# haampie/Homogenization.jl

Hardware: AMD Instinct MI355X
Metric: fine-DOF updates/sec per V-cycle (3D Tet64) (higher is better)
Workload: dtype f64; 1 GPU; 3D Tet64 checkerboard, 32^3 unit cubes x 6 tets, refinements=5 (BASELINE config 3); cells=196608, nf=6545, levels=6, smoothing_steps=3, smoothing_steps_coarse=2, coarse_solver=device CG, Chebyshev(4)-of-Jacobi preconditioner, rtol 1e-13, spare_vector_bytes=10294394880, lazy_top_form=2

## Files before the change

homogenization.jl_amd/csrc/hmg_apply.hip:

```cpp
#include "hmg_apply_launch.hpp"
#include "hmg_device.hpp"
#include "hmg_stencil.hpp"

#include <cstdio>
#include <stdexcept>
#include <string>

namespace hmg {

#ifdef HMG_PHASE_TIMING
#define HMG_STAMP(i)                                                                     \
    do {    \
        if (a.blockpart && !a.cell_list && tid == 0)                                     \
            a.blockpart[2 * (size_t)a.nwork + 8 * cell + (i)] = (double)wall_clock64(); \
    } while (0)
#define HMG_SLAB_T0() const long long _t0 = wall_clock64(); long long _tl = _t0; double _ph[5] = {0, 0, 0, 0, 0}
#define HMG_SLAB_PHASE(i)                              \
    do {                                               \
        const long long _n = wall_clock64();           \
        _ph[i] += (double)(_n - _tl);                  \
        _tl = _n;                                      \
    } while (0)
#define HMG_SLAB_STORE()                                                                      \
    do {                                                                                      \
// ... 1083 lines not shown
    throw std::runtime_error("operator apply: no instantiation for this shape and role");
}

void launch_apply(const Launch &L, const LevelDev &lv, const MeshDev &mesh, double alpha, double lambda,
                  const double *x, const double *src, double *out, int use_mask)
{
    ApplyArgs a{};
    a.alpha = alpha;
    a.lambda = lambda;
    a.x = x;
    a.src = src;
    a.out = out;
    a.flags = (use_mask ? 1 : 0) | (L.apply_mass_only ? 2 : 0);
#ifdef HMG_PHASE_TIMING
    a.blockpart = mesh.blockpart;
#endif
    if (lv.dim == 3)
        launch_apply_dim<3, false>(L, lv, mesh, a);
    else
        launch_apply_dim<2, false>(L, lv, mesh, a);
}

void launch_apply_args(const Launch &L, const LevelDev &lv, const MeshDev &mesh, ApplyArgs a)
{
    a.flags = (a.flags & 1) | (L.apply_mass_only ? 2 : 0);
    if (lv.dim == 3)
        launch_apply_dim<3, false>(L, lv, mesh, a);
    else
        launch_apply_dim<2, false>(L, lv, mesh, a);
}

void launch_apply_fused_kernel(const Launch &L, const LevelDev &lv, const MeshDev &mesh, ApplyArgs a)
{
    a.scal = L.scal;
    if (!(a.flags & 32)) a.mult = mesh.mult;
    a.blockpart = mesh.blockpart;
    if (a.flags & 8) {
        if (lv.dim == 3)
            launch_apply_dim<3, true, true>(L, lv, mesh, a);
        else
            launch_apply_dim<2, true, true>(L, lv, mesh, a);
        return;
    }
    if (lv.dim == 3)
        launch_apply_dim<3, true>(L, lv, mesh, a);
    else
        launch_apply_dim<2, true>(L, lv, mesh, a);
}

void launch_apply_fused_reduce(const Launch &L, const MeshDev &mesh, int slot_pap, int slot_rr)
{
    hipLaunchKernelGGL(k_reduce_pairs, dim3(256), dim3(256), 0, L.stream, mesh.blockpart, mesh.ncells, L.partials);
    check_launch();
    launch_finalize(L, L.partials, 256, slot_pap);
    if (slot_rr >= 0)
        launch_finalize(L, L.partials + 2048, 256, slot_rr);
    check_launch();
}

void launch_restrict_slab(const Launch &L, const LevelDev &fine_rtab, const MeshDev &mesh, const SlabTables &st,
                          int ldc, const double *rf, double *bc)
{
    ApplyArgs a{};
    a.alpha = 1.0;
    a.x = rf;
    a.out = bc;
    a.out_ld = ldc;
// ... 35 lines not shown
```

homogenization.jl_amd/csrc/hmg_context.cpp:

```cpp
#include "../../include/hmg.h"
#include "hmg_objects.hpp"

#include <algorithm>

namespace hmg {

std::recursive_mutex &lifetime_mutex()
{
    static std::recursive_mutex m;
    return m;
}

std::atomic<int64_t> &device_allocs()
{
    static std::atomic<int64_t> n{0};
    return n;
}

namespace {

void vec_pool_trim(hmg_ctx *c)
{
    LifetimeLock lock(lifetime_mutex());
    if (c->vec_pool.empty()) return;
// ... 78 lines not shown
    c->L.rpart_cap = need_blocks;
}

void ctx_unref(hmg_ctx *ctx)
{
    LifetimeLock lock(lifetime_mutex());
    if (!ctx || --ctx->refs > 0) return;
    auto &lc = live_contexts();
    lc.erase(std::remove(lc.begin(), lc.end(), ctx), lc.end());
    (void)hipSetDevice(ctx->device);
    (void)hipStreamSynchronize(ctx->stream);
    for (auto &ev : ctx->timer.pool) {
        (void)hipEventDestroy(ev.first);
        (void)hipEventDestroy(ev.second);
    }
    vec_pool_trim(ctx);
    comm_drop(ctx);
    if (ctx->own_stream) (void)hipStreamDestroy(ctx->stream);
    delete ctx;
}

}

void grid_unref(hmg_grid *grid)
{
    LifetimeLock lock(lifetime_mutex());
    if (!grid || --grid->refs > 0) return;
    hmg_ctx *c = grid->ctx;
    if (c) {
        (void)hipSetDevice(c->device);
        (void)hipStreamSynchronize(c->stream);
    }
    probe_unlist(grid);
    release_top_spare(grid);
    release_weight_cache(grid);
    release_smoother_diag(grid);
    if (grid->probe && grid->probe->h) (void)hipHostFree(grid->probe->h);
    if (grid->probe && grid->probe->ev) (void)hipEventDestroy(grid->probe->ev);
    delete grid;
    ctx_unref(c);
}

void release_vec(hmg_vec *v)
{
    if (v->own && v->d) vec_release(v->g->ctx, v->d, v->bytes);
    hmg_grid *g = v->g;
    delete v;
    grid_unref(g);
}

double read_scalar(hmg_ctx *c, int slot)
{
    double h = 0.0;
    HIPCHK(hipMemcpyAsync(&h, c->L.scal + slot, sizeof(double), hipMemcpyDeviceToHost, c->stream));
    HIPCHK(hipStreamSynchronize(c->stream));
    judge_probes(c);
    return h;
}

}

extern "C" {

const char *hmg_last_error(void) { return last_error().c_str(); }
int hmg_version(void) { return 1; }

// ... 66 lines not shown
int hmg_ctx_sync(hmg_ctx *ctx)
{
    HMG_TRY
    need(ctx != nullptr, "null ctx");
    HIPCHK(hipStreamSynchronize(ctx->stream));
    judge_probes(ctx);
    HMG_END
}

int64_t hmg_ctx_counter(hmg_ctx *ctx, const char *name)
{
    if (!ctx || !name) return -1;
    const std::string n(name);
    if (n == "wave_launches") return ctx->wave_launches;
    if (n == "slab2_launches") return ctx->slab2_launches;
    if (n == "rows_launches") return ctx->rows_launches;
    if (n == "small_launches") return ctx->small_launches;
    if (n == "weight_cache_launches") return ctx->wc_launches;
    if (n == "comm_calls") return ctx->comm_calls;
    if (n == "device_allocs") return device_allocs().load();
    if (n == "spare_bytes") return ctx->spare_bytes;
    if (n == "weight_cache_classes") return ctx->wc_classes;
    if (n == "weight_cache_bytes") return ctx->wc_bytes;
    if (n == "weight_cache_refusals") return ctx->wc_refusals;
    if (n == "fcg_bytes") return ctx->fcg_bytes;
    if (n == "smoother_diag_bytes") return ctx->smoother_diag_bytes;
    if (n == "smoother_diag_builds") return ctx->smoother_diag_builds;
    if (n == "lazy_top_form") return ctx->last_top_form;
    if (n == "lazy_pre_form") return ctx->last_pre_form;
    if (n == "lazy_r_form") return ctx->last_r_form;
    if (n == "r_materialized") return ctx->r_materialized;
    if (n == "r_materialized_by_read") return ctx->r_materialized_read;
    if (n == "r_dropped") return ctx->r_dropped;
    if (n == "coarse_x_folds") return ctx->coarse_x_folds;
    if (n == "cell_moments_kernel_ns") return ctx->moments_kernel_ns;
    if (n == "cell_moments_download_ns") return ctx->moments_download_ns;
    if (n == "cell_pair_moments_kernel_ns") return ctx->pair_moments_kernel_ns;
    if (n == "cell_pair_moments_download_ns") return ctx->pair_moments_download_ns;
    if (n == "cell_moments_window_launches") return ctx->moments_window_launches;
    if (n == "cell_moments_windows") return ctx->moments_windows;
    if (n == "cell_extrema_kernel_ns") return ctx->extrema_kernel_ns;
    if (n == "cell_extrema_window_launches") return ctx->extrema_window_launches;
    if (n == "cell_extrema_windows") return ctx->extrema_windows;
    if (n == "comm_nranks") return ctx->comm ? ctx->comm_nranks : 0;
    return -1;
}

int hmg_ctx_release_memory(hmg_ctx *ctx)
{
    HMG_TRY
    need(ctx != nullptr, "null ctx");
    vec_pool_trim(ctx);
    HMG_END
}

int hmg_ctx_set_option(hmg_ctx *ctx, const char *name, int64_t value)
{
    HMG_TRY
    need(ctx && name, "null argument");
    std::string n(name);
    static const std::pair<const char *, bool hmg_ctx::*> flags[] = {
        {"coarse_probe", &hmg_ctx::coarse_probe}, {"fuse_cg", &hmg_ctx::fuse_cg_default}, {"fold_x", &hmg_ctx::fold_x},
        {"swap_rp", &hmg_ctx::swap_rp}, {"fold_prolong", &hmg_ctx::fold_prolong}, {"zero_entry", &hmg_ctx::zero_entry},
        {"fold_restrict", &hmg_ctx::fold_restrict}, {"lazy_dead", &hmg_ctx::lazy_dead}, {"lazy_pre", &hmg_ctx::lazy_pre}, {"fold_coarse_x", &hmg_ctx::fold_coarse_x}, {"fold_faces", &hmg_ctx::fold_faces},
        {"lean_post", &hmg_ctx::lean_post}, {"lazy_post", &hmg_ctx::lazy_post}, {"lazy_r", &hmg_ctx::lazy_r}, {"prolong_in_image", &hmg_ctx::prolong_in_image},
        {"comm_rehearsal", &hmg_ctx::comm_rehearsal}};
    for (const auto &f : flags)
        if (n == f.first) {
            ctx->*f.second = value != 0;
            return 0;
        }
    if (n == "apply_threads")
        ctx->L.apply_threads = (int)value;
    else if (n == "apply_wg512")
        ctx->L.apply_wg512 = value != 0;
    else if (n == "apply_pack")
        ctx->L.apply_pack = value != 0;
    else if (n == "apply_small")
        ctx->L.apply_small = value != 0;
    else if (n == "weight_cache")
        ctx->L.weight_cache = value != 0;
    else if (n == "weight_cache_classes")
        ctx->wc_max_classes = std::max<int64_t>(0, value);
    else if (n == "apply_slab2")
        ctx->L.apply_slab2 = value != 0;
    else if (n == "restrict_slab2")
        ctx->L.restrict_slab2 = value != 0;
    else if (n == "slab2_force")
        ctx->L.slab2_force = value != 0;
    else if (n == "slab2_grid")
        ctx->L.slab2_grid = std::max<int64_t>(0, value);
    else if (n == "apply_wave")
        ctx->L.apply_wave = value != 0;
    else if (n == "wave_grid")
        ctx->L.wave_grid = std::max<int64_t>(1, value) * (int64_t)ctx->L.num_cu;
    else if (n == "wave_grid_total")
        ctx->L.wave_grid = std::max<int64_t>(1, value);
    else if (n == "cell_order")
// ... 174 lines not shown
```

homogenization.jl_amd/csrc/hmg_kernels.hip:

```cpp
#include "hmg_device.hpp"
#include "hmg_stencil.hpp"

#include <cstdio>
#include <stdexcept>
#include <string>

namespace hmg {

__global__ void __launch_bounds__(256) k_finalize(const double *__restrict__ partials, int n, double *scal, int slot)
{
    __shared__ double red[4];
    double v = 0.0;
    for (int i = threadIdx.x; i < n; i += 256) v += partials[i];
    double s = block_sum(v, red);
    if (threadIdx.x == 0) scal[slot] = s;
}

void launch_finalize(const Launch &L, const double *partials, int n, int slot)
{
    hipLaunchKernelGGL(k_finalize, dim3(1), dim3(256), 0, L.stream, partials, n, L.scal, slot);
}

__global__ void __launch_bounds__(256)
k_iface_faces(const int32_t *__restrict__ pairs, int64_t npairs, int nfi, int off_face, int ld, double *x)
// ... 556 lines not shown
    }
    const double s = block_sum(acc, red);
    if (threadIdx.x == 0) partials[blockIdx.x] = s;
}

template <int XU>
__global__ void __launch_bounds__(SB)
k_cg_x_tail(double *x, const double *__restrict__ p, const double *__restrict__ p0, const double *__restrict__ r, int64_t n,
            const double *__restrict__ scal, int s_num, int s_den, XUSlots xs, double *alpha_out)
{
    static_assert(XU == 1 || XU == 2, "one or two stored directions");
    const double alpha = scal[s_num] / scal[s_den];
    const double ax = scal[xs.a_num] / scal[xs.a_den];
    const double beta = scal[xs.b_num] / scal[xs.b_den];
    const double az = XU == 2 ? scal[xs.z_num] / scal[xs.z_den] : 0.0;
    const int64_t i = (int64_t)blockIdx.x * SB + threadIdx.x;
    if (i < (n >> 1)) {
        double2 xv = reinterpret_cast<double2 *>(x)[i];
        const double2 pv = reinterpret_cast<const double2 *>(p)[i];
        const double2 rv = reinterpret_cast<const double2 *>(r)[i];
        if (XU == 2) {
            const double2 zv = reinterpret_cast<const double2 *>(p0)[i];
            xv.x = axpy1(az, zv.x, xv.x);
            xv.y = axpy1(az, zv.y, xv.y);
        }
        xv.x = xupd2(ax, beta, alpha, xv.x, pv.x, rv.x);
        xv.y = xupd2(ax, beta, alpha, xv.y, pv.y, rv.y);
        reinterpret_cast<double2 *>(x)[i] = xv;
    }
    if (blockIdx.x == 0 && threadIdx.x == 0) {
        if (n & 1) x[n - 1] = xupd2(ax, beta, alpha, XU == 2 ? axpy1(az, p0[n - 1], x[n - 1]) : x[n - 1], p[n - 1], r[n - 1]);
        alpha_out[0] = alpha;
        alpha_out[1] = 1.0;
    }
}

__global__ void __launch_bounds__(SB)
k_cg_xp_update(double *x, double *p, const double *__restrict__ r, int64_t n, const double *__restrict__ scal,
               int a_num, int a_den, int s_num, int s_den, int with_p)
{
    const double alpha = scal[a_num] / scal[a_den];
    const double beta = with_p ? scal[s_num] / scal[s_den] : 0.0;
    const int64_t i = (int64_t)blockIdx.x * SB + threadIdx.x;
    if (i < (n >> 1)) {
        double2 *x2 = reinterpret_cast<double2 *>(x);
        double2 *p2 = reinterpret_cast<double2 *>(p);
        double2 xv = x2[i], pv = p2[i];
        double2 rv = make_double2(0.0, 0.0);
        if (with_p) rv = reinterpret_cast<const double2 *>(r)[i];
        xv.x = axpy1(alpha, pv.x, xv.x);
        xv.y = axpy1(alpha, pv.y, xv.y);
        x2[i] = xv;
        if (with_p) {
            pv.x = axpy1(beta, pv.x, rv.x);
            pv.y = axpy1(beta, pv.y, rv.y);
            p2[i] = pv;
        }
    }
    if ((n & 1) && blockIdx.x == 0 && threadIdx.x == 0) {
        x[n - 1] = axpy1(alpha, p[n - 1], x[n - 1]);
        if (with_p) p[n - 1] = axpy1(beta, p[n - 1], r[n - 1]);
    }
}

__global__ void __launch_bounds__(SB)
k_cg_x2_update(double *x, const double *__restrict__ p, const double *__restrict__ r, int64_t n, const double *__restrict__ scal,
// ... 740 lines not shown
```

homogenization.jl_amd/csrc/hmg_objects.hpp:

```cpp
#pragma once

#include "../../include/hmg.h"
#include "hmg_device.hpp"
#include "hmg_host.hpp"

#include <atomic>
#include <memory>
#include <mutex>
#include <stdexcept>
#include <string>
#include <vector>

struct ncclComm;

using namespace hmg;

#define HIPCHK(expr)                                                                            \
    do {                                                                                        \
        hipError_t _e = (expr);                                                                 \
        if (_e != hipSuccess)                                                                   \
            throw std::runtime_error(std::string("HIP error: ") + hipGetErrorString(_e) + " (" #expr ")"); \
    } while (0)

namespace hmg {
// ... 112 lines not shown
    std::vector<double> ev_bytes;
    size_t used = 0;
};

struct FieldState {
    std::vector<ElementTables> elem;
    std::vector<std::unique_ptr<DevBuf<uint8_t>>> d_mask;
};

struct CoarseProbe {
    double *h = nullptr;
    hipEvent_t ev = nullptr;
    bool pending = false;
    int budget = 0;
    int generation = 0;
};

}

struct hmg_ctx {
    int refs = 1;
    ApplyTimer timer;
    bool fuse_cg_default = true;
    bool fold_x = true;
    bool swap_rp = true;
    bool fold_prolong = true;
    bool lazy_dead = true;
    bool lazy_pre = true;
    bool fold_faces = true;
    bool lean_post = true;
    bool lazy_post = true;
    bool fold_coarse_x = true;
    bool lazy_r = true;
    int lazy_top = 2;
    bool zero_entry = true;
    bool fold_restrict = true;
    bool prolong_in_image = true;
    int device = 0;
    hipStream_t stream = nullptr;
    bool own_stream = false;
    DevBuf<double> partials, scal, rpart;
    Launch L{};
    int coarse_maxit = 5000;
    int coarse_check = 25;
    bool coarse_probe = true;
    double coarse_rtol = 1e-13;
    int coarse_poly = 4;
    double coarse_poly_ratio = 20.0;
    ncclComm *comm = nullptr;
    int comm_nranks = 1, comm_rank = 0;
    hipStream_t comm_stream = nullptr;
    hipEvent_t ev_packed = nullptr, ev_summed = nullptr;
    int64_t comm_calls = 0, comm_doubles = 0;
    int64_t small_launches = 0;
    int64_t wc_launches = 0;
    int64_t wave_launches = 0;
    int64_t slab2_launches = 0;
    int64_t rows_launches = 0;
    int64_t wc_max_classes = 0;
    int64_t wc_classes = 0, wc_bytes = 0;
    int64_t wc_refusals = 0;
    int64_t spare_bytes = 0;
    int64_t fcg_bytes = 0;
    int64_t smoother_diag_bytes = 0;
    int64_t smoother_diag_builds = 0;
    int64_t moments_kernel_ns = 0, moments_download_ns = 0;
    int64_t pair_moments_kernel_ns = 0, pair_moments_download_ns = 0;
    int64_t extrema_kernel_ns = 0;
    int moments_windows = 0;
    int64_t moments_window_launches = 0;
    int extrema_windows = 0;
    int64_t extrema_window_launches = 0;
    int64_t coarse_x_folds = 0;
    int last_pre_form = 0;
    int last_r_form = 0;
    int64_t r_materialized = 0;
    int64_t r_materialized_read = 0;
    int64_t r_dropped = 0;
    int last_top_form = 0;
    bool vec_pool_on = true;
    std::vector<std::pair<size_t, void *>> vec_pool;
    bool comm_rehearsal = false;
    int64_t overlap_min_doubles = 524288;
    std::vector<struct hmg_grid *> probe_grids;
};

struct PendingR {
    hmg_vec *r = nullptr, *Ap = nullptr;
    int level = 0;
    int slot = -1;
    bool formed = false;
    bool orphan_Ap = false;
};

struct hmg_grid {
    int refs = 1;
    hmg_ctx *ctx = nullptr;
    int dim = 0, nlevels = 0;
    std::vector<LevelTables> lt;
    std::vector<std::unique_ptr<LevelBufs>> lb;
    std::vector<LevelDev> ld;
    MeshTables mesh_full, mesh;
    bool shrunk = false;
    bool dir_custom = false;
    std::vector<int32_t> dir_faces;
    MeshDev md{};
    DevBuf<int32_t> d_cells, d_face_pairs, d_face_partner, d_edge_ptr, d_edge_ent, d_node_ptr, d_node_ent, d_node_first;
    DevBuf<uint16_t> d_dmask, d_dupmask;
    DevBuf<uint8_t> d_mult;
    DevBuf<double> d_blockpart;
    PendingR pend;
    bool r_reader = false;
    double *pend_alpha() const { return d_blockpart.p ? d_blockpart.p + d_blockpart.n - 2 : nullptr; }
    bool fuse_cg = true;
    DevBuf<double> d_coef;
    std::vector<double> sigma, coef;
    int sig_n = 0;
    DevBuf<int32_t> d_cell_class;
    DevBuf<double> d_coef_rep;
    int nclasses = 0;
    std::vector<int32_t> cell_class;
    int64_t wc_limit = 0;
    bool wc_trim = false;
    int64_t wc_counted_classes = 0, wc_counted_bytes = 0;
    double wc_lambda = 0.0;
    bool wc_ready = false;
    double lambda = 0.0;
    bool has_op = false;
    uint64_t op_epoch = 0;
    CoarseMatrix cm;
    CoarseDev cd{};
    bool coarse_ready = false;
    DevBuf<int32_t> c_rowptr, c_colidx, c_interior;
    DevBuf<double> c_val, c_diag, c_b, c_x, c_r, c_z, c_p, c_q, c_u, c_z2, c_d;
    DevBuf<double> top_spare;
    bool top_spare_refused = false;
    int smoother = 0;
    std::vector<std::unique_ptr<DevBuf<double>>> dinv;
    bool dinv_ready = false;
    std::vector<char> dinv_level_ready;
    bool dinv_build_counted = false;
    double c_lmax = 2.0;
    int coarse_last_it = 0;
    int coarse_budget = 0;
    int coarse_generation = 0;
    int64_t coarse_misses = 0;
// ... 48 lines not shown
{
    last_error() = e.what();
    return 1;
}

#define HMG_TRY try {
#define HMG_END                      \
    }                                \
    catch (const std::exception &e)  \
    {                                \
        return fail(e);              \
    }                                \
    catch (...)                      \
    {                                \
        last_error() = "unknown error"; \
        return 1;                    \
    }                                \
    return 0;

inline void need(bool c, const char *msg)
{
    if (!c) throw std::runtime_error(msg);
}

inline const LevelDev &lev(const hmg_grid *g, int level)
{
    need(g != nullptr, "null grid");
    need(g->ctx != nullptr, "this grid was created without a device context (host tables only): no compute path exists on the CPU");
    need(level >= 1 && level <= g->nlevels, "level out of range");
    return g->ld[level - 1];
}

void materialize_r(hmg_grid *g, bool read = false);
inline void settle(const hmg_vec *v)
{
    if (v && v->g && v->g->pend.r && (v == v->g->pend.r || v == v->g->pend.Ap)) materialize_r(v->g, true);
}
void settle_overwritten(const hmg_vec *v);
bool pending_keeps(hmg_vec *v);

inline void check_vec(const hmg_grid *g, int level, const hmg_vec *v, const char *name, bool settle_pending = true)
{
    if (!v) throw std::runtime_error(std::string("null vector: ") + name);
    if (v->g != g) throw std::runtime_error(std::string("vector belongs to another grid: ") + name);
    if (v->level != level) throw std::runtime_error(std::string("vector has the wrong level: ") + name);
    if (v->alloc_cells < g->md.ncells) throw std::runtime_error(std::string("vector too small: ") + name);
    if (settle_pending) settle(v);
}

inline int64_t vec_len(const hmg_vec *v) { return (int64_t)v->g->ld[v->level - 1].ld * v->g->md.ncells; }

inline bool has_exchange(const hmg_grid *g) { return g->exchange || g->ex_begin || g->p2p || g->p2p_begin; }

double *vec_alloc(hmg_ctx *c, size_t bytes);
void vec_release(hmg_ctx *c, void *p, size_t bytes);
void release_vec(hmg_vec *v);
void grid_unref(hmg_grid *grid);
double read_scalar(hmg_ctx *c, int slot);

void ensure_weight_cache(hmg_grid *g);
void release_weight_cache(hmg_grid *g);

SlabTables slab_tables(const hmg_grid *g, const LevelDev &lv);

void set_slab(hmg_grid *g, const LevelDev &lv);
void apply(hmg_grid *g, const LevelDev &lv, double alpha, const double *x, const double *src, double *out, int mask);
// ... 24 lines not shown
```

homogenization.jl_amd/csrc/hmg_smooth.cpp:

```cpp
#include "../../include/hmg.h"
#include "hmg_objects.hpp"
#include "hmg_pcg.hpp"

#include <algorithm>
#include <cmath>

namespace hmg {

void set_slab(hmg_grid *g, const LevelDev &lv)
{
    const LevelBufs &B = *g->lb[lv.level - 1];
    g->md.slab.head = B.slab_head.p;
    g->md.slab.ld_word = B.slab_ld_word.p;
    g->md.slab.cp_word = B.slab_cp_word.p;
    g->md.slab.cp_slot = B.slab_cp_slot.p;
    g->md.slab.nslab = B.nslab;
    g->md.slab.lds_nodes = B.slab_lds_nodes;
    g->md.slab.max_surf = B.slab_max_surf;
    g->md.slab.max_int = B.slab_max_int;
}

namespace {

struct TimedRegion {
// ... 397 lines not shown
            a.out = Ap->d;
            a.flags = 1;
            apply_then_sum(g, lv, a, true, S_PAP, -1);
        } else {
            apply(g, lv, 1.0, p->d, nullptr, Ap->d, 1);
            interface_sum(g, lv, Ap->d);
            launch_dot(L, p->d, Ap->d, n, S_PAP);
            scalar_sum(g, S_PAP, 1);
        }
        const bool last = i == steps - 1;
        if (last && f.tail != Tail::Full) {
            if (f.tail == Tail::ScratchP) {
                launch_pcg_rupdate(L, r->d, Ap->d, dinv, n, cur, S_PAP, other);
                scalar_sum(g, other, 1);
            }
            launch_cg_xp_update(L, x->d, p->d, r->d, n, cur, S_PAP, cur, other, 0);
            return;
        }
        launch_pcg_rupdate(L, r->d, Ap->d, dinv, n, cur, S_PAP, other);
        scalar_sum(g, other, 1);
        launch_pcg_xp(L, x->d, p->d, r->d, dinv, n, cur, S_PAP, other, cur);
        std::swap(cur, other);
    }
}

bool lazy_r_ok(const hmg_grid *g, const hmg_vec *r, const hmg_vec *p, const hmg_vec *Ap)
{
    if (!g->ctx->lazy_r || g->smoother != 0 || g->part || has_exchange(g) || g->scalar_sum) return false;
    for (const hmg_vec *v : {r, p, Ap})
        if (!v->own || v->exposed) return false;
    return r != Ap && g->pend_alpha() != nullptr && vec_len(r) > 0;
}

void open_pending(hmg_grid *g, int level, hmg_vec *r, hmg_vec *Ap, int slot, bool formed)
{
    LifetimeLock lock(lifetime_mutex());
    need(!g->pend.r, "a pending r-update was not settled before the next one");
    g->pend.r = r;
    g->pend.Ap = Ap;
    g->pend.level = level;
    g->pend.slot = slot;
    g->pend.formed = formed;
    g->ctx->last_r_form = formed ? 0 : 1;
}

DeferredX smooth(hmg_grid *g, int level, int steps, hmg_vec *x, hmg_vec *b, hmg_vec *r, hmg_vec *p, hmg_vec *Ap,
                 const SmoothForm &f, const hmg_vec *xcoarse = nullptr, const DeferredX *cx = nullptr)
{
    const LevelDev &lv = lev(g, level);
    const Launch &L = g->ctx->L;
    const int64_t n = vec_len(x);
    first_residual(g, level, x, b, r, f, xcoarse, cx);
    if (g->smoother == 1) {
        smooth_pcg(g, level, steps, x, r, p, Ap, f);
        return {};
    }
    int cur = S_RS, other = S_RS2;
    if (!g->fuse_cg || steps <= 0) {
        launch_copy_dot(L, p->d, r->d, n, cur);
        scalar_sum(g, cur, 1);
        for (int i = 0; i < steps; ++i) {
            apply(g, lv, 1.0, p->d, nullptr, Ap->d, 1);
            interface_sum(g, lv, Ap->d);
            launch_dot(L, p->d, Ap->d, n, S_PAP);
            scalar_sum(g, S_PAP, 1);
            const bool last = i == steps - 1;
            if (last && f.tail == Tail::DeadXp) {
                launch_cg_xp_update(L, x->d, p->d, r->d, n, cur, S_PAP, cur, other, 0);
                return {};
            }
            launch_cg_update(L, x->d, r->d, p->d, Ap->d, n, cur, S_PAP, other);
            scalar_sum(g, other, 1);
            if (last && f.tail == Tail::ScratchP) return {};
            launch_cg_pupdate(L, p->d, r->d, n, other, cur);
            std::swap(cur, other);
        }
        return {};
    }
    auto args = [&](int i) {
        ApplyArgs a{};
        a.alpha = 1.0;
        a.lambda = g->lambda;
        a.x = r->d;
        a.x2 = i == 0 ? nullptr : p->d;
// ... 72 lines not shown
        }
        return DeferredX{cur, S_PAP2, true, other, S_PAP, cur, other};
    case Tail::DeadDefer3:
        a.x2 = g->top_spare.p;
        a.out = a.xout = a.xacc = nullptr;
        a.s_num = S_RS3;
        a.s_den = cur;
        apply_then_sum(g, lv, a, true, S_PAP3, -1);
        {
            DeferredX d{S_RS3, S_PAP3, true, cur, S_PAP2, S_RS3, cur};
            d.three_updates = true;
            d.d_num = other;
            d.d_den = S_PAP;
            return d;
        }
    case Tail::Top2:
        a.xout = a.xacc = nullptr;
        apply_then_sum(g, lv, a, true, S_PAP2, -1, true, false);
        if (f.lazy_r && !g->r_reader) {
            launch_cg_x_tail(L, r->d, n, cur, S_PAP2, x->d, p->d, other, S_PAP, cur, other, nullptr, 0, 0, g->pend_alpha());
            open_pending(g, level, r, Ap, other, false);
            return {};
        }
        launch_cg_rupdate_faces_x(L, lv, g->md, r->d, r->d, Ap->d, n, cur, S_PAP2, other, x->d, p->d, other, S_PAP, cur, other,
                                  nullptr, 0, 0);
        scalar_sum(g, other, 1);
        if (f.lazy_r) open_pending(g, level, r, Ap, other, true);
        return {};
    case Tail::Top3:
        a.x2 = g->top_spare.p;
        a.xout = a.xacc = nullptr;
        a.s_num = S_RS3;
        a.s_den = cur;
        apply_then_sum(g, lv, a, true, S_PAP3, -1, true, false);
        if (f.lazy_r && !g->r_reader) {
            launch_cg_x_tail(L, r->d, n, S_RS3, S_PAP3, x->d, g->top_spare.p, cur, S_PAP2, S_RS3, cur, p->d, other, S_PAP, g->pend_alpha());
            open_pending(g, level, r, Ap, other, false);
            return {};
        }
        launch_cg_rupdate_faces_x(L, lv, g->md, r->d, r->d, Ap->d, n, S_RS3, S_PAP3, other, x->d, g->top_spare.p, cur, S_PAP2,
                                  S_RS3, cur, p->d, other, S_PAP);
        scalar_sum(g, other, 1);
        if (f.lazy_r) open_pending(g, level, r, Ap, other, true);
        return {};
    }
    return {};
}

bool zero_entry_ok(const hmg_grid *g, int k, int steps)
{
    if (!g->ctx->zero_entry) return false;
    if (k == 1) return true;
    if (g->smoother == 1) return false;
    if (steps != 2 || smooth_form(g, k, steps, Role::Pre).tail != Tail::DeadDefer2) return false;
    const LevelDev &lv = g->ld[k - 1];
    if (lv.blk_R > 0) return g->ctx->fold_restrict && apply_restricts(g->ctx->L, lv);
    return true;
}

int vcycle_down(hmg_grid *g, int k, int steps, hmg_vec **st, bool inside = false, bool x_zero = false, int steps_next = -1)
{
    hmg_vec **cur = st + 5 * (k - 1);
    hmg_vec **nxt = st + 5 * (k - 2);
    const Launch &L = g->ctx->L;
    SmoothForm form = smooth_form(g, k, steps, Role::Pre);
    need(!x_zero || form.tail == Tail::DeadDefer2, "zero initial guess: the pre-smoother does not defer both x-updates");
// ... 55 lines not shown
    const bool fold_p = g->ctx->fold_prolong && g->fuse_cg && apply_lds_bytes(lev(g, k)) <= 160 * 1024 &&
                        apply_lds_bytes(lev(g, k)) + sizeof(double) * (size_t)lev(g, k - 1).nf <= 80 * 1024;
    need(!(cx && cx->rs >= 0) || fold_p, "pending coarse x-updates without the folded prolongation");
    if (!fold_p) launch_prolong_add(L, lev(g, k), lev(g, k - 1), g->md.ncells, nxt[0]->d, cur[0]->d);
    SmoothForm form = smooth_form(g, k, steps, role);
    form.hand_up = hand_up && form.tail == Tail::DeadX2;
    form.lazy_r = lazy_r && (form.tail == Tail::Top2 || form.tail == Tail::Top3) && lazy_r_ok(g, cur[2], cur[3], cur[4]);
    return smooth(g, k, steps, cur[0], cur[1], cur[2], cur[3], cur[4], form, fold_p ? nxt[0] : nullptr, cx);
}

bool coarse_x_folds(const hmg_grid *g, int k, int steps_below)
{
    const hmg_ctx *c = g->ctx;
    if (k < 3 || g->smoother == 1 || !c->fold_coarse_x || !c->lazy_post || !c->fold_prolong || !c->lean_post || !g->fuse_cg || !c->prolong_in_image) return false;
    const LevelDev &lv = g->ld[(size_t)k - 1];
    if (!(apply_lds_bytes(lv) > 48 * 1024 && apply_lds_bytes(lv) <= 160 * 1024 &&
          apply_lds_bytes(lv) + sizeof(double) * (size_t)g->ld[(size_t)k - 2].nf <= 80 * 1024))
        return false;
    return apply_folds_coarse_x(c->L, lv) && smooth_form(g, k - 1, steps_below, Role::PostBelow).tail == Tail::DeadX2;
}

DeferredX vcycle_level(hmg_grid *g, int k, int steps, int steps_coarse, hmg_vec **st, bool top, bool zero_guess, bool hand_up)
{
    if (k == 1) {
        hmg_vec **cur = st;
        coarse_solve(g, cur[1], cur[0]);
        return {};
    }
    const bool x_zero = (zero_guess || !top) && zero_entry_ok(g, k, steps);
    if (top && zero_guess && !x_zero) launch_fill(g->ctx->L, st[5 * (k - 1)]->d, vec_len(st[5 * (k - 1)]), 0.0);
    const int deferred = vcycle_down(g, k, steps, st, true, x_zero, steps_coarse);
    if (top) g->ctx->last_pre_form = deferred;
    const DeferredX cx = vcycle_level(g, k - 1, steps_coarse, steps_coarse, st, false, false, coarse_x_folds(g, k, steps_coarse));
    if (top) g->ctx->last_top_form = g->ctx->last_r_form = 0;
    return vcycle_up(g, k, steps, st, top ? Role::PostTop : Role::PostBelow, &cx, hand_up, top);
}

}

namespace {

void close_pending(hmg_grid *g)
{
    hmg_vec *orphan = g->pend.orphan_Ap ? g->pend.Ap : nullptr;
    g->pend = PendingR{};
    if (orphan) release_vec(orphan);
}

void drop_pending(hmg_grid *g)
{
    if (!g->pend.formed) g->ctx->r_dropped += 1;
    g->r_reader = false;
    close_pending(g);
}

}

void materialize_r(hmg_grid *g, bool read)
{
    LifetimeLock lock(lifetime_mutex());
    const PendingR q = g->pend;
    if (!q.r) return;
    if (!q.formed) {
        HIPCHK(hipSetDevice(g->ctx->device));
        launch_cg_rupdate_faces(g->ctx->L, lev(g, q.level), g->md, q.r->d, q.r->d, q.Ap->d, vec_len(q.r), 0, 1, q.slot, g->pend_alpha());
        g->ctx->r_materialized += 1;
        if (read) g->ctx->r_materialized_read += 1;
    }
    close_pending(g);
    if (read) g->r_reader = true;
}

void settle_overwritten(const hmg_vec *v)
{
    if (!v || !v->g || !v->g->pend.r) return;
    LifetimeLock lock(lifetime_mutex());
    hmg_grid *g = v->g;
    if (v == g->pend.Ap)
        materialize_r(g);
    else if (v == g->pend.r)
        drop_pending(g);
}

bool pending_keeps(hmg_vec *v)
{
    hmg_grid *g = v->g;
    if (!g || !g->pend.r) return false;
    if (v == g->pend.r)
        drop_pending(g);
    else if (v == g->pend.Ap) {
        if (!g->pend.formed) {
            g->pend.orphan_Ap = true;
            return true;
        }
        close_pending(g);
    }
    return false;
// ... 270 lines not shown
```

homogenization.jl_amd/csrc/hmg_upload.cpp:

```cpp
#include "../../include/hmg.h"
#include "hmg_objects.hpp"

#include <cmath>
#include <cstdlib>
#include <cstring>
#include <unordered_map>

namespace hmg {
namespace {

void upload_mesh(hmg_grid *g)
{
    const MeshTables &M = g->cur();
    const char *xcd_env = std::getenv("HMG_XCD_LISTS");
    const MeshKernelTables K = build_mesh_kernel_tables(M, !(xcd_env && xcd_env[0] == '0'));
    DryUploads dry_scope(!g->ctx, &g->upload_hash);
    hipStream_t s = g->ctx ? g->ctx->stream : nullptr;
    g->d_cells.upload(M.cells, s);
    g->d_face_pairs.upload(M.face_pairs, s);
    g->d_face_partner.upload(K.face_partner, s);
    g->d_edge_ptr.upload(M.edge_ptr, s);
    g->d_edge_ent.upload(M.edge_ent, s);
    g->d_node_ptr.upload(M.node_ptr, s);
    g->d_node_ent.upload(M.node_ent, s);
    g->d_node_first.upload(M.node_first, s);
    g->d_dmask.upload(K.dmask, s);
    g->d_dupmask.upload(M.dupmask, s);
    g->d_mult.upload(M.mult, s);
#ifdef HMG_PHASE_TIMING
    constexpr size_t BP = 10;
#else
    constexpr size_t BP = 2;
#endif
    if (g->d_blockpart.n < (size_t)M.ncells * BP + 2) g->d_blockpart.alloc((size_t)M.ncells * BP + 2);
    g->d_cells_cut.upload(K.cells_cut, s);
    g->d_cells_inner.upload(K.cells_inner, s);
    g->d_cell_perm.upload(K.cell_perm, s);
    MeshDev &d = g->md;
    d.dim = M.dim;
    d.ncells = M.ncells;
    d.nnodes = M.nnodes;
    d.cells = g->d_cells.p;
    d.face_pairs = g->d_face_pairs.p;
    d.face_partner = g->d_face_partner.p;
    d.nfacepairs = (int64_t)M.face_pairs.size() / 3;
    d.edge_ptr = g->d_edge_ptr.p;
    d.edge_ent = g->d_edge_ent.p;
    d.nsharededges = (int64_t)M.edge_ptr.size() - 1;
    d.node_ptr = g->d_node_ptr.p;
    d.node_ent = g->d_node_ent.p;
    d.nsharednodes = (int64_t)M.node_ptr.size() - 1;
    d.node_first = g->d_node_first.p;
    d.dmask = g->d_dmask.p;
    d.dupmask = g->d_dupmask.p;
    d.mult = g->d_mult.p;
    d.blockpart = g->d_blockpart.p;
    d.cells_cut = g->d_cells_cut.p;
    d.cells_inner = g->d_cells_inner.p;
    d.ncells_cut = (int64_t)M.cells_cut.size();
    d.ncells_inner = (int64_t)M.cells_inner.size();
    d.cell_perm = g->d_cell_perm.p;
    d.ncut_edge_groups = M.ncut_edge_groups;
    d.ncut_node_groups = M.ncut_node_groups;
    d.ncut_face_pairs = M.ncut_face_pairs;
    d.coef = g->d_coef.p;
}

// ... 316 lines not shown
    }
    upload_levels(g.get());
    upload_mesh(g.get());
    if (part) finish_partition(g.get());
    if (ctx) {
        LifetimeLock lock(lifetime_mutex());
        ctx->refs += 1;
    }
    *out = g.release();
    HMG_END
}

int hmg_grid_create(hmg_ctx *ctx, int dim, int nlevels, int64_t nnodes, const double *coords, int64_t ncells,
                    const int64_t *cells, hmg_grid **out)
{
    return create_grid(ctx, dim, nlevels, nnodes, coords, ncells, cells, false, nullptr, nullptr, 0, 1, out);
}

int hmg_grid_create_partition(hmg_ctx *ctx, int dim, int nlevels, int64_t nnodes, const double *coords, int64_t ncells,
                              const int64_t *cells, const int32_t *owner, int rank, int nranks, hmg_grid **out)
{
    return create_grid(ctx, dim, nlevels, nnodes, coords, ncells, cells, true, owner, nullptr, rank, nranks, out);
}

int hmg_grid_create_partition_rehearsal(hmg_ctx *ctx, int dim, int nlevels, int64_t nnodes, const double *coords,
                                        int64_t ncells, const int64_t *cells, const int32_t *owner, const int32_t *cut_owner,
                                        int rank, int nranks, hmg_grid **out)
{
    return create_grid(ctx, dim, nlevels, nnodes, coords, ncells, cells, true, owner, cut_owner, rank, nranks, out);
}

static void set_operator(hmg_grid *g, const double *sigma, int sn, double lambda)
{
    if (g->part)
        g->sigma_global.assign(sigma, sigma + (size_t)g->part->global.ncells * sn);
    else
        g->sigma.assign(sigma, sigma + (size_t)g->mesh_full.ncells * sn);
    g->sig_n = sn;
    g->wc_limit = g->ctx ? g->ctx->wc_max_classes : 0;
    g->wc_trim = true;
    g->lambda = lambda;
    g->has_op = true;
    g->op_epoch += 1;
    g->dinv_ready = false;
    upload_operator(g);
}

int hmg_grid_set_operator(hmg_grid *g, const double *sigma, double lambda)
{
    HMG_TRY
    need(g && sigma, "null argument");
    set_operator(g, sigma, g->dim, lambda);
    HMG_END
}

int hmg_grid_set_operator_tensor(hmg_grid *g, const double *sigma, double lambda)
{
    HMG_TRY
    need(g && sigma, "null argument");
    const int dim = g->dim, nc = sym_ncomp(dim);
    const int64_t n = g->part ? g->part->global.ncells : g->mesh_full.ncells;
    bool diagonal = true;
    for (int64_t c = 0; c < n; ++c) {
        const double *s = sigma + (size_t)c * nc;
        for (int t = 0; t < nc; ++t)
            if (!std::isfinite(s[t])) throw std::runtime_error("sigma of cell " + std::to_string(c) + " is not finite");
        bool spd;
        if (dim == 2) {
            spd = s[0] > 0.0 && s[0] * s[2] - s[1] * s[1] > 0.0;
            diagonal = diagonal && s[1] == 0.0;
        } else {
            const double m2 = s[0] * s[3] - s[1] * s[1];
            const double m3 = s[0] * (s[3] * s[5] - s[4] * s[4]) - s[1] * (s[1] * s[5] - s[4] * s[2]) + s[2] * (s[1] * s[4] - s[3] * s[2]);
            spd = s[0] > 0.0 && m2 > 0.0 && m3 > 0.0;
            diagonal = diagonal && s[1] == 0.0 && s[2] == 0.0 && s[4] == 0.0;
        }
        if (!spd) throw std::runtime_error("sigma of cell " + std::to_string(c) + " is not positive definite");
    }
    if (diagonal) {
        std::vector<double> d((size_t)n * dim);
        for (int64_t c = 0; c < n; ++c)
            for (int a = 0; a < dim; ++a) d[(size_t)c * dim + a] = sigma[(size_t)c * nc + sym_index(dim, a, a)];
        set_operator(g, d.data(), dim, lambda);
    } else {
        set_operator(g, sigma, nc, lambda);
    }
    HMG_END
}

int hmg_grid_set_lambda(hmg_grid *g, double lambda)
{
    HMG_TRY
    need(g != nullptr, "null grid");
    g->lambda = lambda;
    g->op_epoch += 1;
    g->dinv_ready = false;
    g->coarse_ready = false;
    if (g->ctx && g->has_op) ensure_weight_cache(g);
    HMG_END
}

int hmg_grid_shrink(hmg_grid *g, int64_t ncells_prefix, int64_t nnodes_prefix)
{
    HMG_TRY
    need(g != nullptr, "null grid");
    need(!g->dir_custom, "hmg_grid_shrink: the grid holds a caller's Dirichlet faces (hmg_grid_set_dirichlet_faces); restore the "
                         "default set first (nfaces = -1)");
    if (g->ctx) materialize_r(g);
    g->op_epoch += 1;
    g->dinv_ready = false;
    if (g->part) {
        need(ncells_prefix >= 1 && ncells_prefix <= g->part_ncells && nnodes_prefix >= 1 && nnodes_prefix <= g->part_nnodes,
             "prefix out of range");
        const int rank = g->part->rank, nranks = g->part->nranks;
        std::unique_ptr<Partition> np(new Partition);
        MeshTables local;
        build_partition(g->dim, nnodes_prefix, g->part_coords.data(), ncells_prefix, g->part_cells.data(),
                        g->part_owner.data(), rank, nranks, local, *np,
                        g->part_cut_owner.empty() ? nullptr : g->part_cut_owner.data(), g->part_halo);
        need(local.ncells <= g->mesh_full.ncells, "shrunk partition is larger than the original one");
        g->mesh = std::move(local);
        g->part = std::move(np);
        g->shrunk = true;
        upload_mesh(g);
        finish_partition(g);
        if (g->has_op) upload_operator(g);
// ... 257 lines not shown
```

Baseline: 11.93 billion fine-DOF updates/s.

## Defer storing Ap in final top-level smoother step; rebuild lazily on materialize

In the last Top3 smoothing step with lazy r, the operator apply no longer writes Ap to memory. It only computes the p·Ap reduction, and the pending r-update records that Ap was not stored. If r is later materialized, Ap is recomputed from r and the top spare vector using saved scalars, which are stored in two extra blockpart slots. The intent is to save a full fine-level vector write per V-cycle when the pending r is dropped. The cost is an extra operator apply whenever r must actually be formed, plus settle hooks on option, operator and lambda changes and on grid release.

```diff
diff --git a/homogenization.jl_amd/csrc/hmg_apply.hip b/homogenization.jl_amd/csrc/hmg_apply.hip
--- a/homogenization.jl_amd/csrc/hmg_apply.hip
+++ b/homogenization.jl_amd/csrc/hmg_apply.hip
@@ -1139,7 +1139,7 @@
 
 void launch_apply_fused_kernel(const Launch &L, const LevelDev &lv, const MeshDev &mesh, ApplyArgs a)
 {
-    a.scal = L.scal;
+    if (!a.scal) a.scal = L.scal;
     if (!(a.flags & 32)) a.mult = mesh.mult;
     a.blockpart = mesh.blockpart;
     if (a.flags & 8) {
diff --git a/homogenization.jl_amd/csrc/hmg_context.cpp b/homogenization.jl_amd/csrc/hmg_context.cpp
--- a/homogenization.jl_amd/csrc/hmg_context.cpp
+++ b/homogenization.jl_amd/csrc/hmg_context.cpp
@@ -134,6 +134,9 @@
         (void)hipStreamSynchronize(c->stream);
     }
     probe_unlist(grid);
+    if (c) {
+        c->pend_grids.erase(std::remove(c->pend_grids.begin(), c->pend_grids.end(), grid), c->pend_grids.end());
+    }
     release_top_spare(grid);
     release_weight_cache(grid);
     release_smoother_diag(grid);
@@ -266,6 +269,8 @@
     if (n == "r_materialized") return ctx->r_materialized;
     if (n == "r_materialized_by_read") return ctx->r_materialized_read;
     if (n == "r_dropped") return ctx->r_dropped;
+    if (n == "lazy_ap_form") return ctx->last_ap_form;
+    if (n == "ap_rebuilt") return ctx->ap_rebuilt;
     if (n == "coarse_x_folds") return ctx->coarse_x_folds;
     if (n == "cell_moments_kernel_ns") return ctx->moments_kernel_ns;
     if (n == "cell_moments_download_ns") return ctx->moments_download_ns;
@@ -293,11 +298,16 @@
     HMG_TRY
     need(ctx && name, "null argument");
     std::string n(name);
+    {
+        LifetimeLock lock(lifetime_mutex());
+        const std::vector<hmg_grid *> open = ctx->pend_grids;
+        for (hmg_grid *g : open) settle_rebuild(g);
+    }
     static const std::pair<const char *, bool hmg_ctx::*> flags[] = {
         {"coarse_probe", &hmg_ctx::coarse_probe}, {"fuse_cg", &hmg_ctx::fuse_cg_default}, {"fold_x", &hmg_ctx::fold_x},
         {"swap_rp", &hmg_ctx::swap_rp}, {"fold_prolong", &hmg_ctx::fold_prolong}, {"zero_entry", &hmg_ctx::zero_entry},
         {"fold_restrict", &hmg_ctx::fold_restrict}, {"lazy_dead", &hmg_ctx::lazy_dead}, {"lazy_pre", &hmg_ctx::lazy_pre}, {"fold_coarse_x", &hmg_ctx::fold_coarse_x}, {"fold_faces", &hmg_ctx::fold_faces},
-        {"lean_post", &hmg_ctx::lean_post}, {"lazy_post", &hmg_ctx::lazy_post}, {"lazy_r", &hmg_ctx::lazy_r}, {"prolong_in_image", &hmg_ctx::prolong_in_image},
+        {"lean_post", &hmg_ctx::lean_post}, {"lazy_post", &hmg_ctx::lazy_post}, {"lazy_r", &hmg_ctx::lazy_r}, {"lazy_ap", &hmg_ctx::lazy_ap}, {"prolong_in_image", &hmg_ctx::prolong_in_image},
         {"comm_rehearsal", &hmg_ctx::comm_rehearsal}};
     for (const auto &f : flags)
         if (n == f.first) {
diff --git a/homogenization.jl_amd/csrc/hmg_kernels.hip b/homogenization.jl_amd/csrc/hmg_kernels.hip
--- a/homogenization.jl_amd/csrc/hmg_kernels.hip
+++ b/homogenization.jl_amd/csrc/hmg_kernels.hip
@@ -612,6 +612,8 @@
         if (n & 1) x[n - 1] = xupd2(ax, beta, alpha, XU == 2 ? axpy1(az, p0[n - 1], x[n - 1]) : x[n - 1], p[n - 1], r[n - 1]);
         alpha_out[0] = alpha;
         alpha_out[1] = 1.0;
+        alpha_out[2] = scal[xs.b_num];
+        alpha_out[3] = scal[xs.b_den];
     }
 }
 
diff --git a/homogenization.jl_amd/csrc/hmg_objects.hpp b/homogenization.jl_amd/csrc/hmg_objects.hpp
--- a/homogenization.jl_amd/csrc/hmg_objects.hpp
+++ b/homogenization.jl_amd/csrc/hmg_objects.hpp
@@ -168,6 +168,7 @@
     bool lazy_post = true;
     bool fold_coarse_x = true;
     bool lazy_r = true;
+    bool lazy_ap = true;
     int lazy_top = 2;
     bool zero_entry = true;
     bool fold_restrict = true;
@@ -213,12 +214,15 @@
     int64_t r_materialized = 0;
     int64_t r_materialized_read = 0;
     int64_t r_dropped = 0;
+    int last_ap_form = 0;
+    int64_t ap_rebuilt = 0;
     int last_top_form = 0;
     bool vec_pool_on = true;
     std::vector<std::pair<size_t, void *>> vec_pool;
     bool comm_rehearsal = false;
     int64_t overlap_min_doubles = 524288;
     std::vector<struct hmg_grid *> probe_grids;
+    std::vector<struct hmg_grid *> pend_grids;
 };
 
 struct PendingR {
@@ -226,6 +230,7 @@
     int level = 0;
     int slot = -1;
     bool formed = false;
+    bool ap_stored = true;
     bool orphan_Ap = false;
 };
 
@@ -247,7 +252,7 @@
     DevBuf<double> d_blockpart;
     PendingR pend;
     bool r_reader = false;
-    double *pend_alpha() const { return d_blockpart.p ? d_blockpart.p + d_blockpart.n - 2 : nullptr; }
+    double *pend_alpha() const { return d_blockpart.p ? d_blockpart.p + d_blockpart.n - 4 : nullptr; }
     bool fuse_cg = true;
     DevBuf<double> d_coef;
     std::vector<double> sigma, coef;
@@ -362,6 +367,10 @@
 }
 
 void materialize_r(hmg_grid *g, bool read = false);
+inline void settle_rebuild(hmg_grid *g)
+{
+    if (g && g->ctx && g->pend.r && !g->pend.ap_stored) materialize_r(g);
+}
 inline void settle(const hmg_vec *v)
 {
     if (v && v->g && v->g->pend.r && (v == v->g->pend.r || v == v->g->pend.Ap)) materialize_r(v->g, true);
diff --git a/homogenization.jl_amd/csrc/hmg_smooth.cpp b/homogenization.jl_amd/csrc/hmg_smooth.cpp
--- a/homogenization.jl_amd/csrc/hmg_smooth.cpp
+++ b/homogenization.jl_amd/csrc/hmg_smooth.cpp
@@ -453,16 +453,26 @@
     return r != Ap && g->pend_alpha() != nullptr && vec_len(r) > 0;
 }
 
-void open_pending(hmg_grid *g, int level, hmg_vec *r, hmg_vec *Ap, int slot, bool formed)
+void open_pending(hmg_grid *g, int level, hmg_vec *r, hmg_vec *Ap, int slot, bool formed, bool ap_stored = true)
 {
     LifetimeLock lock(lifetime_mutex());
     need(!g->pend.r, "a pending r-update was not settled before the next one");
+    need(ap_stored || !formed, "a formed r-update without its Ap");
     g->pend.r = r;
     g->pend.Ap = Ap;
     g->pend.level = level;
     g->pend.slot = slot;
     g->pend.formed = formed;
+    g->pend.ap_stored = ap_stored;
     g->ctx->last_r_form = formed ? 0 : 1;
+    g->ctx->last_ap_form = ap_stored ? 0 : 1;
+    auto &open = g->ctx->pend_grids;
+    if (std::find(open.begin(), open.end(), g) == open.end()) open.push_back(g);
+}
+
+bool lazy_ap_ok(const hmg_grid *g, const SmoothForm &f)
+{
+    return g->ctx->lazy_ap && f.tail == Tail::Top3 && f.lazy_r && !g->r_reader;
 }
 
 DeferredX smooth(hmg_grid *g, int level, int steps, hmg_vec *x, hmg_vec *b, hmg_vec *r, hmg_vec *p, hmg_vec *Ap,
@@ -471,6 +481,7 @@
     const LevelDev &lv = lev(g, level);
     const Launch &L = g->ctx->L;
     const int64_t n = vec_len(x);
+    if (f.tail == Tail::Top3 || f.tail == Tail::DeadDefer3) settle_rebuild(g);
     first_residual(g, level, x, b, r, f, xcoarse, cx);
     if (g->smoother == 1) {
         smooth_pcg(g, level, steps, x, r, p, Ap, f);
@@ -609,6 +620,13 @@
         a.xout = a.xacc = nullptr;
         a.s_num = S_RS3;
         a.s_den = cur;
+        if (lazy_ap_ok(g, f)) {
+            a.out = nullptr;
+            apply_then_sum(g, lv, a, true, S_PAP3, -1);
+            launch_cg_x_tail(L, r->d, n, S_RS3, S_PAP3, x->d, g->top_spare.p, cur, S_PAP2, S_RS3, cur, p->d, other, S_PAP, g->pend_alpha());
+            open_pending(g, level, r, Ap, other, false, false);
+            return {};
+        }
         apply_then_sum(g, lv, a, true, S_PAP3, -1, true, false);
         if (f.lazy_r && !g->r_reader) {
             launch_cg_x_tail(L, r->d, n, S_RS3, S_PAP3, x->d, g->top_spare.p, cur, S_PAP2, S_RS3, cur, p->d, other, S_PAP, g->pend_alpha());
@@ -730,7 +748,7 @@
     const int deferred = vcycle_down(g, k, steps, st, true, x_zero, steps_coarse);
     if (top) g->ctx->last_pre_form = deferred;
     const DeferredX cx = vcycle_level(g, k - 1, steps_coarse, steps_coarse, st, false, false, coarse_x_folds(g, k, steps_coarse));
-    if (top) g->ctx->last_top_form = g->ctx->last_r_form = 0;
+    if (top) g->ctx->last_top_form = g->ctx->last_r_form = g->ctx->last_ap_form = 0;
     return vcycle_up(g, k, steps, st, top ? Role::PostTop : Role::PostBelow, &cx, hand_up, top);
 }
 
@@ -742,6 +760,10 @@
 {
     hmg_vec *orphan = g->pend.orphan_Ap ? g->pend.Ap : nullptr;
     g->pend = PendingR{};
+    if (g->ctx) {
+        auto &open = g->ctx->pend_grids;
+        open.erase(std::remove(open.begin(), open.end(), g), open.end());
+    }
     if (orphan) release_vec(orphan);
 }
 
@@ -761,6 +783,22 @@
     if (!q.r) return;
     if (!q.formed) {
         HIPCHK(hipSetDevice(g->ctx->device));
+        if (!q.ap_stored) {
+            need(g->top_spare.p != nullptr && g->pend_alpha() != nullptr, "a pending r-update has lost the spare vector it rests on");
+            const LevelDev &lv = lev(g, q.level);
+            ApplyArgs a{};
+            a.alpha = 1.0;
+            a.lambda = g->lambda;
+            a.x = q.r->d;
+            a.x2 = g->top_spare.p;
+            a.out = q.Ap->d;
+            a.scal = g->pend_alpha();
+            a.s_num = 2;
+            a.s_den = 3;
+            a.flags = 1;
+            apply_then_sum(g, lv, a, true, S_PAP3, -1, true, false);
+            g->ctx->ap_rebuilt += 1;
+        }
         launch_cg_rupdate_faces(g->ctx->L, lev(g, q.level), g->md, q.r->d, q.r->d, q.Ap->d, vec_len(q.r), 0, 1, q.slot, g->pend_alpha());
         g->ctx->r_materialized += 1;
         if (read) g->ctx->r_materialized_read += 1;
diff --git a/homogenization.jl_amd/csrc/hmg_upload.cpp b/homogenization.jl_amd/csrc/hmg_upload.cpp
--- a/homogenization.jl_amd/csrc/hmg_upload.cpp
+++ b/homogenization.jl_amd/csrc/hmg_upload.cpp
@@ -32,7 +32,7 @@
 #else
     constexpr size_t BP = 2;
 #endif
-    if (g->d_blockpart.n < (size_t)M.ncells * BP + 2) g->d_blockpart.alloc((size_t)M.ncells * BP + 2);
+    if (g->d_blockpart.n < (size_t)M.ncells * BP + 4) g->d_blockpart.alloc((size_t)M.ncells * BP + 4);
     g->d_cells_cut.upload(K.cells_cut, s);
     g->d_cells_inner.upload(K.cells_inner, s);
     g->d_cell_perm.upload(K.cell_perm, s);
@@ -415,6 +415,7 @@
 
 static void set_operator(hmg_grid *g, const double *sigma, int sn, double lambda)
 {
+    settle_rebuild(g);
     if (g->part)
         g->sigma_global.assign(sigma, sigma + (size_t)g->part->global.ncells * sn);
     else
@@ -475,6 +476,7 @@
 {
     HMG_TRY
     need(g != nullptr, "null grid");
+    settle_rebuild(g);
     g->lambda = lambda;
     g->op_epoch += 1;
     g->dinv_ready = false;
```

Result: faster. 12.12 billion fine-DOF updates/s (median of 6 runs) (+1.6%).
